# zxhuang1698/ShapeClipper

Measured on AMD Instinct MI355X. Metric: train-step images/sec (Pix3D cfg, bs32/GPU), higher is better.
Workload: dtype f32 (bf16x3-split MFMA, fp32 accumulate)

## Files before the change

### include/shapeclipper_hip.h

```cpp
#ifndef SHAPECLIPPER_HIP_H
#define SHAPECLIPPER_HIP_H
#include <stdint.h>
#ifdef __cplusplus
extern "C" {
#endif

int sc_chamfer3d_forward(const float* xyz1, const float* xyz2, float* dist1, float* dist2,
                         int32_t* idx1, int32_t* idx2, int b, int n, int m, void* stream);

int sc_chamfer3d_forward_split(const float* xyz1, const float* xyz2, float* dist1, float* dist2,
                               int32_t* idx1, int32_t* idx2, int b, int n, int m, int nsplit,
                               void* workspace, void* stream);

long long sc_chamfer3d_grid_workspace_bytes(int b, int n, int m);
int sc_chamfer3d_forward_grid(const float* xyz1, const float* xyz2, float* dist1, float* dist2,
                              int32_t* idx1, int32_t* idx2, int b, int n, int m, void* workspace, void* stream);

int sc_chamfer3d_backward(const float* xyz1, const float* xyz2, float* gradxyz1, float* gradxyz2,
                          const float* graddist1, const float* graddist2, const int32_t* idx1,
                          const int32_t* idx2, int b, int n, int m, void* stream);

long long sc_chamfer3d_backward_ordered_workspace_bytes(int b, int n, int m);
int sc_chamfer3d_backward_ordered_chunk(void);
int sc_chamfer3d_backward_ordered(const float* xyz1, const float* xyz2, float* gradxyz1, float* gradxyz2,
// ... 370 lines not shown
int sc_conv3x3_tile_channels(int hw);
int sc_conv3x3_pack_multi(const long long* table, int n, float* dst, long long total, void* stream);
int sc_conv3x3_pack_multi_units(const long long* table, int n, float* dst, long long total, void* stream);
int sc_conv3x3_pack(const float* w, float* w_pack, int cin, int cout, int hw, int transpose_flip, void* stream);
int sc_conv3x3_forward(const float* x, const float* w_pack, float* out, float* workspace, int batch, int cin, int cout, int hw,
                       void* stream);

long long sc_conv3x3_pack_floats_split(int cin, int cout, int hw);
long long sc_conv3x3_workspace_floats_split(int hw);
int sc_conv3x3_tile_channels_split(int hw);
int sc_conv3x3_forward_split(const float* x, const float* w_pack, float* out, float* workspace, int batch, int cin, int cout, int hw,
                             void* stream);
int sc_conv3x3_forward_add(const float* x, const float* w_pack, const float* addend, float* out, float* workspace, int batch, int cin,
                           int cout, int hw, int split, void* stream);

long long sc_conv3x3s2_bd_pack_floats(int cin, int cout, int hw);
long long sc_conv3x3s2_bd_workspace_floats(int hw);
int sc_conv3x3s2_bd_pack(const float* w, float* w_pack, int cin, int cout, int hw, void* stream);
int sc_conv3x3s2_backward_data(const float* gy, const float* w_pack, float* gx, float* workspace, int batch, int cin, int cout, int hw,
                               void* stream);
int sc_conv3x3s2_wgrad(const float* gy, const float* x, float* dw, float* workspace, int batch, int cin, int cout, int hw, void* stream);
long long sc_conv3x3s2_pack_floats(int cin, int cout, int hw);
long long sc_conv3x3s2_workspace_floats(int hw);
int sc_conv3x3s2_forward(const float* x, const float* w_pack, float* out, float* workspace, int batch, int cin, int cout, int hw,
                         void* stream);

long long sc_conv3x3_wgrad_workspace_floats(int cin, int cout);
int sc_conv3x3_wgrad(const float* gy, const float* x, float* dw, float* workspace, int batch, int cin, int cout, int hw, void* stream);
int sc_conv3x3_wgrad_split(const float* gy, const float* x, float* dw, float* workspace, int batch, int cin, int cout, int hw, void* stream);

long long sc_conv_stem_wgrad_workspace_floats(void);
int sc_conv_stem_forward(const float* x, const float* w, float* out, int batch, void* stream);
int sc_conv_stem_wgrad(const float* gy, const float* x, float* dw, float* workspace, int batch, void* stream);

long long sc_conv1x1s2_wgrad_workspace_floats(int cin, int cout);
int sc_conv1x1s2_forward(const float* x, const float* w, float* out, int batch, int cin, int cout, int hin, void* stream);
int sc_conv1x1s2_backward_data(const float* gy, const float* w, float* gx, int batch, int cin, int cout, int hin, void* stream);
int sc_conv1x1s2_wgrad(const float* gy, const float* x, float* dw, float* workspace, int batch, int cin, int cout, int hin, void* stream);

typedef struct sc_block_args {
    const float *x, *pf1, *pf2, *pb1, *pb2;
    const float *g1, *b1, *g2, *b2;
    float *rm1, *rv1, *rm2, *rv2;
    int64_t *nt1, *nt2;
    float *y1, *a1, *y2, *out, *st1, *st2;
    float *conv_ws, *bn_ws, *wgrad_ws;
    const float* d_out;
    float *dy2, *dres, *da1, *dy1, *dx, *gw1, *gw2, *dgb1, *dgb2;
    int batch, channels, hw, groups, training, split, need_dx;
    float mom1, eps1, mom2, eps2;
} sc_block_args;
int sc_basic_block_forward(const sc_block_args* args, void* stream);
int sc_basic_block_backward(const sc_block_args* args, void* stream);

int sc_linear_bn_supported(int N, int Cin, int Cout, int groups);
int sc_linear_bn_forward(const float* x, const float* w, const float* gamma, const float* beta, const float* res, float* y, float* out,
                         float* save_mean, float* save_rstd, float* run_mean, float* run_var, int64_t* n_tracked, int N, int Cin,
                         int Cout, int groups, int training, int relu, float eps, float momentum, void* stream);
int sc_linear_bn_backward(const float* g_out, const float* gy_next, const float* w_next, const float* g_add, int Cnext, const float* out,
                          const float* y, const float* save_mean, const float* save_rstd, const float* gamma, const float* x, float* gy,
                          float* g_res, float* dw, float* dgamma, float* dbeta, int N, int Cin, int Cout, int groups, int training, int relu,
                          void* stream);
int sc_linear_backward_data(const float* gy, const float* w, const float* g_add, float* dx, int N, int Cin, int Cout, void* stream);

int sc_latent_bias_forward(const float* z, const float* lat, const float* bias, const float* post, float* out, int B, int Z, int L, int NL,
                           void* stream);
// ... 49 lines not shown
```

### shapeclipper_amd/_lib.py

```python
from __future__ import annotations

import ctypes
import os
import re
import threading
from typing import Optional

import torch

_HERE = os.path.dirname(os.path.abspath(__file__))
LIB_PATH = os.environ.get("SHAPECLIPPER_HIP_LIB") or os.path.join(_HERE, "lib", "libshapeclipper_hip.so")

HEADER_PATH = os.path.join(_HERE, os.pardir, "include", "shapeclipper_hip.h")
_CTYPES = {"int": ctypes.c_int, "long long": ctypes.c_longlong, "float": ctypes.c_float, "double": ctypes.c_double}


def read_signatures(text):
    text = re.sub(r"/\*.*?\*/|//[^\n]*", " ", text, flags=re.S)
    text = re.sub(r"^[ \t]*#.*$", " ", text, flags=re.M)
    text = re.sub(r"typedef struct sc_block_args \{.*?\} sc_block_args", " ", text, flags=re.S)
    text = re.sub(r'extern "C" \{|\}', " ", text)
    sigs = {}
    for decl in filter(None, (" ".join(d.split()) for d in text.split(";"))):
        m = re.fullmatch(r"(int|long long) (sc_\w+)\((.*)\)", decl)
        if m is None:
            raise RuntimeError("shapeclipper_amd: include/shapeclipper_hip.h: unrecognised declaration %r" % decl)
        params = [] if m.group(3) == "void" else m.group(3).split(",")
        try:
            args = [ctypes.c_void_p if "*" in p else _CTYPES[" ".join(w for w in p.split()[:-1] if w != "const")] for p in params]
        except KeyError:
            raise RuntimeError("shapeclipper_amd: include/shapeclipper_hip.h: unrecognised parameter type in %r" % decl) from None
        sigs[m.group(2)] = (_CTYPES[m.group(1)], args)
    return sigs


with open(HEADER_PATH) as _f:
    SIGNATURES = read_signatures(_f.read())
SYMBOLS = tuple(n for n, (res, _) in SIGNATURES.items() if res is ctypes.c_int)
SYMBOLS_OTHER = tuple(n for n, (res, _) in SIGNATURES.items() if res is ctypes.c_longlong)

_lib: Optional[ctypes.CDLL] = None

TIMING = None
TIMING_SKIP = ("sc_sdf_stream_pack", "sc_sdf_stream_pack_bytes", "sc_rgb_composite_backward_fused_parts", "sc_rgb_composite_backward_fused_partial_floats", "sc_latent_bias_forward", "sc_latent_bias_backward", "sc_set_reserved_cus", "sc_grid_cus", "sc_chamfer3d_backward_ordered_chunk","sc_conv3x3_release_tables", "sc_linear_bn_supported", "sc_linear_bn_forward", "sc_linear_bn_backward", "sc_linear_backward_data", "sc_bn_splits", "sc_isosurface_blocks_per_image", "sc_marching_cubes_mesh_vertex_blocks_per_image", "sc_bn_act_forward", "sc_bn_act_backward", "sc_bn_relu_pool_forward", "sc_bn_relu_pool_backward",
               "sc_conv3x3_forward", "sc_conv3x3_forward_split", "sc_conv3x3_forward_add", "sc_conv3x3_wgrad", "sc_conv3x3_wgrad_split", "sc_conv3x3_pack", "sc_conv3x3_pack_multi", "sc_conv3x3_pack_multi_units",
               "sc_conv_stem_forward", "sc_conv_stem_wgrad", "sc_conv1x1s2_forward", "sc_conv1x1s2_backward_data", "sc_conv1x1s2_wgrad",
               "sc_conv3x3s2_forward", "sc_conv3x3s2_bd_pack", "sc_conv3x3s2_backward_data", "sc_conv3x3s2_wgrad", "sc_conv3x3_tile_channels", "sc_conv3x3_tile_channels_split",
               "sc_basic_block_forward", "sc_basic_block_backward")

class _Timed:

    def __init__(self, name, fn):
        self.name, self.fn = name, fn

    def __call__(self, *args):
        if TIMING is None:
            return self.fn(*args)
        s, e = torch.cuda.Event(enable_timing=True), torch.cuda.Event(enable_timing=True)
        s.record()
        code = self.fn(*args)
        e.record()
        TIMING.setdefault(self.name, []).append((s, e, args))
        return code


class _LibProxy:

    def __init__(self, cdll):
        self._cdll = cdll
        for name, (restype, argtypes) in SIGNATURES.items():
            fn = getattr(cdll, name)
            fn.restype, fn.argtypes = restype, argtypes
            setattr(self, name, _Timed(name, fn) if restype is ctypes.c_int and name not in TIMING_SKIP else fn)


class HipLibraryMissing(RuntimeError):
    pass


# ... 45 lines not shown
```

### shapeclipper_amd/csrc/conv_stem.hip

```cpp
#include <hip/hip_runtime.h>

#include "grid_cus.hpp"
#include "shapeclipper_hip.h"

namespace sc {

typedef float st_f32x16 __attribute__((ext_vector_type(16)));

constexpr int ST_WI = 224, ST_WO = 112, ST_WP = 230, ST_K = 147, ST_KP = 148, ST_CO = 64;
constexpr int ST_HWI = ST_WI * ST_WI, ST_HWO = ST_WO * ST_WO;
constexpr int SF_PT = 256;
constexpr int SF_ROWS = 13;
constexpr int SF_CH = SF_ROWS * ST_WP;
constexpr int SF_PATCH = 3 * SF_CH;
constexpr int SF_WLD = 96;
constexpr int SF_LDS = ST_KP * SF_WLD + SF_PATCH;
constexpr int SF_NLOAD = (3 * SF_ROWS + 7) / 8;

__global__ __launch_bounds__(512, 1) void conv_stem_fwd_kernel(const float* __restrict__ x, const float* __restrict__ w,
                                                               float* __restrict__ out, int batch) {
    extern __shared__ float4 st_smem[];
    float* Ws = reinterpret_cast<float*>(st_smem);
    float* Xs = Ws + ST_KP * SF_WLD;
    const int tid = threadIdx.x, lane = tid & 63, wave = __builtin_amdgcn_readfirstlane(tid >> 6), half = lane >> 5;
    const int tiles = batch * (ST_HWO / SF_PT), G = gridDim.x, g = blockIdx.x;
    const int t_lo = (int)((long long)g * tiles / G), t_hi = (int)((long long)(g + 1) * tiles / G);

    for (int i = tid; i < ST_KP * SF_WLD; i += 512) {
        const int k = i / SF_WLD, co = i - k * SF_WLD;
        Ws[i] = (k < ST_K && co < ST_CO) ? w[co * ST_K + k] : 0.f;
    }

    float xv[SF_NLOAD][4];
// ... 165 lines not shown
#pragma unroll
            for (int nt = 0; nt < 5; ++nt)
#pragma unroll
                for (int r = 0; r < 16; ++r) acc[nt][r] += R[((cot * 5 + nt) * 16 + r) * 64 + lane];
        }
        __syncthreads();
    }
    if (kq == 0) {
        float* dst = partial + (size_t)g * SW_PART;
#pragma unroll
        for (int nt = 0; nt < 5; ++nt)
#pragma unroll
            for (int r = 0; r < 16; ++r) dst[((cot * 5 + nt) * 16 + r) * 64 + lane] = acc[nt][r];
    }
}

__global__ void conv_stem_wgrad_reduce_kernel(const float* __restrict__ partial, float* __restrict__ dw, int G) {
    const int e = blockIdx.x * blockDim.x + threadIdx.x;
    if (e >= SW_PART) return;
    float s0 = 0.f, s1 = 0.f, s2 = 0.f, s3 = 0.f;
    int gi = 0;
    for (; gi + 3 < G; gi += 4) {
        s0 += partial[(size_t)gi * SW_PART + e];
        s1 += partial[(size_t)(gi + 1) * SW_PART + e];
        s2 += partial[(size_t)(gi + 2) * SW_PART + e];
        s3 += partial[(size_t)(gi + 3) * SW_PART + e];
    }
    for (; gi < G; ++gi) s0 += partial[(size_t)gi * SW_PART + e];
    const int lane = e & 63, r = (e >> 6) & 15, nt = (e >> 10) % 5, cot = e / (5 * 1024);
    const int co = 32 * cot + (r & 3) + 8 * (r >> 2) + 4 * (lane >> 5), k = 32 * nt + (lane & 31);
    if (k < ST_K) dw[co * ST_K + k] = (s0 + s1) + (s2 + s3);
}

static int stem_cus() { return grid_cus(); }

}

extern "C" long long sc_conv_stem_wgrad_workspace_floats(void) { return (long long)sc::stem_cus() * sc::SW_PART; }

extern "C" int sc_conv_stem_forward(const float* x, const float* w, float* out, int batch, void* stream) {
    if (batch <= 0) return (int)hipErrorInvalidValue;
    (void)hipFuncSetAttribute((const void*)sc::conv_stem_fwd_kernel, hipFuncAttributeMaxDynamicSharedMemorySize, sc::SF_LDS * 4);
    hipLaunchKernelGGL(sc::conv_stem_fwd_kernel, dim3(sc::stem_cus()), dim3(512), sc::SF_LDS * 4, (hipStream_t)stream, x, w, out, batch);
    return (int)hipGetLastError();
}

extern "C" int sc_conv_stem_wgrad(const float* gy, const float* x, float* dw, float* workspace, int batch, void* stream) {
    if (batch <= 0) return (int)hipErrorInvalidValue;
    const int G = sc::stem_cus();
    (void)hipFuncSetAttribute((const void*)sc::conv_stem_wgrad_kernel, hipFuncAttributeMaxDynamicSharedMemorySize, sc::SW_LDS * 4);
    hipLaunchKernelGGL(sc::conv_stem_wgrad_kernel, dim3(G), dim3(512), sc::SW_LDS * 4, (hipStream_t)stream, gy, x, workspace, batch);
    hipLaunchKernelGGL(sc::conv_stem_wgrad_reduce_kernel, dim3((sc::SW_PART + 255) / 256), dim3(256), 0, (hipStream_t)stream, workspace, dw, G);
    return (int)hipGetLastError();
}
```

### shapeclipper_amd/functional.py

```python
from __future__ import annotations

import torch

from . import ops


class SdfFunction(torch.autograd.Function):

    @staticmethod
    def forward(ctx, points, w_pack, cbias, n_per_image, symmetric, want_grad, want_feat, fused_backward=True):
        ctx.set_materialize_grads(False)
        points = points.contiguous()
        need = any(ctx.needs_input_grad[:3])
        res = ops.sdf_forward(points, w_pack, cbias, n_per_image, symmetric=symmetric, want_grad=want_grad,
                              want_feat=want_feat, stash=need)
        sdf, grad, feat = res[0], res[1], res[2]
        ctx.meta = (n_per_image, cbias.shape[0], symmetric, want_grad, want_feat)
        ctx.fused_backward = fused_backward
        if need:
            ctx.save_for_backward(points, w_pack, res[3], res[4] if want_grad else None)
        empty = points.new_empty(0)
        outs = (sdf, grad if want_grad else empty, feat if want_feat else empty)
        nd = [o for o, w in zip(outs[1:], (want_grad, want_feat)) if not w]
        if nd:
# ... 228 lines not shown
    return BnReluPoolFunction.apply(x, bn.weight, bn.bias, *_bn_state(bn), groups)


class Conv3x3Function(torch.autograd.Function):

    @staticmethod
    def forward(ctx, x, w, pack_f, pack_b, split):
        x = ops._aligned(x)
        ctx.save_for_backward(x, w, pack_b)
        ctx.split = split
        if pack_f is None:
            pack_f = ops.conv3x3_pack(w, x.shape[2], False, split)
        return ops.conv3x3_apply(x, pack_f, w.shape[0], split)

    @staticmethod
    def backward(ctx, gy):
        x, w, pack_b = ctx.saved_tensors
        gy = ops._aligned(gy)
        gx = None
        if ctx.needs_input_grad[0]:
            gx = ops.conv3x3_apply(gy, pack_b if pack_b is not None else ops.conv3x3_pack(w, x.shape[2], True, ctx.split), w.shape[1], ctx.split)
        gw = None
        if ctx.needs_input_grad[1]:
            if ops.conv3x3_wgrad_supported(x.shape, w.shape):
                gw = ops.conv3x3_backward_weight(gy, x, split=ctx.split)
            else:
                gw = torch.ops.aten.convolution_backward(gy, x, w, None, [1, 1], [1, 1], [1, 1], False, [0, 0], 1, [False, True, False])[1]
        return gx, gw, None, None, None


class ConvStemFunction(torch.autograd.Function):

    @staticmethod
    def forward(ctx, x, w):
        x = ops._aligned(x)
        ctx.save_for_backward(x, w)
        return ops.conv_stem_forward(x, w)

    @staticmethod
    def backward(ctx, gy):
        x, w = ctx.saved_tensors
        gy = ops._aligned(gy)
        gx = None
        if ctx.needs_input_grad[0]:
            gx = torch.ops.aten.convolution_backward(gy, x, w, None, [2, 2], [3, 3], [1, 1], False, [0, 0], 1, [True, False, False])[0]
        gw = ops.conv_stem_backward_weight(gy, x) if ctx.needs_input_grad[1] else None
        return gx, gw


def conv_stem(conv, x):
    if (x.is_cuda and x.dtype == torch.float32 and conv.bias is None and conv.groups == 1 and conv.dilation == (1, 1)
            and ops.conv_stem_supported(x.shape, conv.weight.shape, conv.stride, conv.padding)):
        return ConvStemFunction.apply(x, conv.weight)
    return conv(x)


class Conv1x1S2Function(torch.autograd.Function):

    @staticmethod
    def forward(ctx, x, w):
        x = ops._aligned(x)
        ctx.save_for_backward(x, w)
        return ops.conv1x1s2_forward(x, w)

    @staticmethod
    def backward(ctx, gy):
        x, w = ctx.saved_tensors
        gy = ops._aligned(gy)
        gx = ops.conv1x1s2_backward_data(gy, w) if ctx.needs_input_grad[0] else None
        gw = ops.conv1x1s2_backward_weight(gy, x) if ctx.needs_input_grad[1] else None
        return gx, gw


def conv1x1s2(conv, x):
    if (x.is_cuda and x.dtype == torch.float32 and conv.bias is None and conv.groups == 1 and conv.dilation == (1, 1)
            and ops.conv1x1s2_supported(x.shape, conv.weight.shape, conv.stride, conv.padding)):
        return Conv1x1S2Function.apply(x, conv.weight)
    return conv(x)


class Conv3x3S2Function(torch.autograd.Function):

    @staticmethod
    def forward(ctx, x, w):
        x = ops._aligned(x)
        ctx.save_for_backward(x, w)
# ... 200 lines not shown
```

### shapeclipper_amd/model/resnet.py

```python
from __future__ import annotations

import torch
import torch.nn as nn

from ..functional import basic_block, basic_block_takes, bn_act, bn_relu_maxpool, conv1x1s2, conv3x3, conv3x3s2, conv_stem

FUSED_BN = True
HIP_CONV3X3 = True
HIP_CONV_STEM = True
HIP_CONV3X3_S2 = True
HIP_CONV3X3_S2_GRADS = True
HIP_CONV_1X1 = True
FUSED_BLOCK = True
HIP_CONV3X3_SPLIT = True


class BasicBlock(nn.Module):
    expansion = 1

    def __init__(self, inplanes, planes, stride=1, downsample=None):
        super().__init__()
        self.conv1 = nn.Conv2d(inplanes, planes, 3, stride, 1, bias=False)
        self.bn1 = nn.BatchNorm2d(planes)
        self.relu = nn.ReLU(inplace=True)
        self.conv2 = nn.Conv2d(planes, planes, 3, 1, 1, bias=False)
        self.bn2 = nn.BatchNorm2d(planes)
        self.downsample = downsample

    def forward(self, x, groups=1, packs=None, hip_conv=None):
        if not FUSED_BN:
            assert groups == 1
            identity = x if self.downsample is None else self.downsample(x)
            out = self.relu(self.bn1(self.conv1(x)))
            out = self.bn2(self.conv2(out))
            return self.relu(out + identity)
        use_hip = HIP_CONV3X3 if hip_conv is None else hip_conv
        if use_hip and FUSED_BLOCK and basic_block_takes(self, x, packs):
            return basic_block(self, x, packs, groups)
        identity = x if self.downsample is None else bn_act(
            self.downsample[1], conv1x1s2(self.downsample[0], x) if (use_hip and HIP_CONV_1X1) else self.downsample[0](x), relu=False, groups=groups)
        conv = (lambda m, t: conv3x3s2(m, t) if (m.stride == (2, 2) and HIP_CONV3X3_S2) else conv3x3(m, t, packs)) if use_hip else (lambda m, t: m(t))
        out = bn_act(self.bn1, conv(self.conv1, x), groups=groups)
        return bn_act(self.bn2, conv(self.conv2, out), residual=identity, groups=groups)


class ResNet(nn.Module):
    def __init__(self, layers, num_classes=1000):
# ... 91 lines not shown
```

### shapeclipper_amd/ops.py

```python
from __future__ import annotations

import collections
import ctypes
import weakref

import torch

from . import _lib
from .packing import n_tiles

_SCRATCH = {}


def _scratch(tag, dev, n_floats):
    if dev.type != "cuda":
        raise RuntimeError(_lib.NO_CPU)
    key = (tag, dev.index, torch._C._cuda_getCurrentRawStream(dev.index))
    buf = _SCRATCH.get(key)
    if buf is None or buf.numel() < n_floats:
        buf = _SCRATCH[key] = torch.empty(n_floats, device=dev, dtype=torch.float32)
    return buf


SDF_SCRATCH_FLOATS = 256 * 8 * 5 * 1024
# ... 1021 lines not shown
    code = _lib.load().sc_basic_block_forward(ctypes.byref(a), _lib.raw_stream(x.get_device()))
    if code:
        _lib.check(code, "sc_basic_block_forward")
    return out, (y1, a1, y2, st[0], st[1])


def basic_block_backward(d_out, x, saved, out, pb1, pb2, g1, b1, g2, b2, training, split, groups, need_dx, need_w1, need_w2):
    y1, a1, y2, st1, st2 = saved
    B, C, H, _ = x.shape
    dy2, da1, dy1 = (torch.empty_like(x) for _ in range(3))
    dx, dres = (torch.empty_like(x), torch.empty_like(x)) if need_dx else (None, None)
    gw1 = torch.empty(C, C, 3, 3, device=x.device, dtype=torch.float32) if need_w1 else None
    gw2 = torch.empty(C, C, 3, 3, device=x.device, dtype=torch.float32) if need_w2 else None
    dgb = torch.empty(2, 2, C, device=x.device, dtype=torch.float32)
    a = BlockArgs()
    a.x, a.pb1, a.pb2, a.d_out = x.data_ptr(), pb1.data_ptr(), pb2.data_ptr(), d_out.data_ptr()
    a.g1, a.b1, a.g2, a.b2 = g1.data_ptr(), b1.data_ptr(), g2.data_ptr(), b2.data_ptr()
    a.y1, a.a1, a.y2, a.out, a.st1, a.st2 = y1.data_ptr(), a1.data_ptr(), y2.data_ptr(), out.data_ptr(), st1.data_ptr(), st2.data_ptr()
    a.dy2, a.da1, a.dy1, a.dres, a.dx = dy2.data_ptr(), da1.data_ptr(), dy1.data_ptr(), _p(dres), _p(dx)
    a.gw1, a.gw2, a.dgb1, a.dgb2 = _p(gw1), _p(gw2), dgb[0].data_ptr(), dgb[1].data_ptr()
    a.conv_ws, a.bn_ws = _conv_workspace(x.device, H, split).data_ptr(), _bn_partial(x, groups)
    a.wgrad_ws = _wgrad_workspace(x, C, C).data_ptr() if (need_w1 or need_w2) else None
    a.batch, a.channels, a.hw, a.groups, a.training, a.split, a.need_dx = B, C, H, groups, 1 if training else 0, 1 if split else 0, 1 if need_dx else 0
    code = _lib.load().sc_basic_block_backward(ctypes.byref(a), _lib.raw_stream(x.get_device()))
    if code:
        _lib.check(code, "sc_basic_block_backward")
    return dx, gw1, dgb[0, 0], dgb[0, 1], gw2, dgb[1, 0], dgb[1, 1]


def conv_stem_supported(x_shape, w_shape, stride=2, padding=3) -> bool:
    return (tuple(x_shape[1:]) == (3, 224, 224) and tuple(w_shape) == (64, 3, 7, 7) and stride in (2, (2, 2)) and padding in (3, (3, 3)))


def conv_stem_forward(x, w):
    lib = _lib.load()
    x, w = _aligned(x), _aligned(w)
    out = torch.empty(x.shape[0], 64, 112, 112, device=x.device, dtype=torch.float32)
    _lib.check(lib.sc_conv_stem_forward(_lib.ptr(x), _lib.ptr(w), _lib.ptr(out), x.shape[0], _lib.stream()), "sc_conv_stem_forward")
    return out


def conv_stem_backward_weight(gy, x):
    lib = _lib.load()
    gy, x = _aligned(gy), _aligned(x)
    ws = _scratch("conv stem", x.device, lib.sc_conv_stem_wgrad_workspace_floats())
    dw = torch.empty(64, 3, 7, 7, device=x.device, dtype=torch.float32)
    _lib.check(lib.sc_conv_stem_wgrad(_lib.ptr(gy), _lib.ptr(x), _lib.ptr(dw), _lib.ptr(ws), x.shape[0], _lib.stream()), "sc_conv_stem_wgrad")
    return dw


def conv1x1s2_supported(x_shape, w_shape, stride=2, padding=0) -> bool:
    return (len(x_shape) == 4 and tuple(w_shape[2:]) == (1, 1) and stride in (2, (2, 2)) and padding in (0, (0, 0)) and x_shape[2] == x_shape[3]
            and x_shape[2] % 2 == 0 and w_shape[1] == x_shape[1] and w_shape[0] % 64 == 0 and w_shape[1] % 64 == 0)


def conv1x1s2_forward(x, w):
    lib = _lib.load()
    x, w = _aligned(x), _aligned(w)
    B, cin, H, _ = x.shape
    out = torch.empty(B, w.shape[0], H // 2, H // 2, device=x.device, dtype=torch.float32)
    _lib.check(lib.sc_conv1x1s2_forward(_lib.ptr(x), _lib.ptr(w), _lib.ptr(out), B, cin, w.shape[0], H, _lib.stream()), "sc_conv1x1s2_forward")
    return out


def conv1x1s2_backward_data(gy, w):
    lib = _lib.load()
    gy, w = _aligned(gy), _aligned(w)
    B, cout, Ho, _ = gy.shape
    gx = torch.empty(B, w.shape[1], 2 * Ho, 2 * Ho, device=gy.device, dtype=torch.float32)
    _lib.check(lib.sc_conv1x1s2_backward_data(_lib.ptr(gy), _lib.ptr(w), _lib.ptr(gx), B, w.shape[1], cout, 2 * Ho, _lib.stream()),
               "sc_conv1x1s2_backward_data")
    return gx


def conv1x1s2_backward_weight(gy, x):
    lib = _lib.load()
    gy, x = _aligned(gy), _aligned(x)
    B, cin, H, _ = x.shape
    cout = gy.shape[1]
    n = lib.sc_conv1x1s2_wgrad_workspace_floats(cin, cout)
# ... 886 lines not shown
```

### shapeclipper_amd/utils/options.py

```python
from __future__ import annotations

import collections
import importlib
import os
import random
import string
import sys

import numpy as np
import torch
import yaml

from . import util
from .util import EasyDict as edict
from .util import log

torch.backends.cudnn.benchmark = False

Switch = collections.namedtuple("Switch", ["key", "default", "kind", "text", "drives"])
HIP_TABLE = tuple(Switch(*row) for row in (
    ("device_rng", False, bool, "draw the render's jitter on the GPU (no 4 MB upload per render, another random stream than the reference)", None),
    ("device_choice", True, bool, "pick the regularisation view on the device (reg.n_views = 1)", None),
    ("device_rays", True, bool, "Pix3D: silhouette-weighted ray choice for the whole batch on the GPU (csrc/silhouette_rays.hip)", None),
    ("device_clip_preprocess", True, bool, "Pix3D: CLIP preprocessing on the GPU (csrc/clip_preprocess.hip)", None),
# ... 3 lines not shown
    ("fused_adam", True, bool, "torch's fused Adam on the device", None),
    ("guarded_step", True, bool, "a non-finite loss skips the update on the device; the host raises one step later", None),
    ("batched_encoders", True, bool, "one grouped encoder pass and one grouped estimator pass per step", None),
    ("two_streams", True, bool, "the view estimator runs on a side stream next to the encoders", None),
    ("overlap_allreduce", False, bool, "multi-GPU: the early gradient segment is all-reduced from inside backward", None),
    ("reserve_cus", 0, (0, None), "multi-GPU: persistent convolution grids sized for the device's CUs minus this many", None),
    ("fused_block", True, bool, "one autograd node per stride-1 BasicBlock", ("model.resnet", "FUSED_BLOCK")),
    ("fused_bottleneck", True, bool, "1x1 Bottleneck_Linear blocks as fused launches (csrc/bottleneck.hip)", ("model.view_estimator", "HIP_BOTTLENECK")),
    ("fused_rgb_wgrad", True, bool, "RGB reverse pass forms the weight gradients in the kernel; off: Gy_l / r_l through HBM and sc_wgrad",
     ("ops", "FUSED_RGB_WGRAD")),
    ("rgb_stash", True, bool, "RGB forward parks its hidden activations for the reverse pass; off: the reverse pass recomputes them",
     ("ops", "RGB_STASH")),
    ("value_split", True, bool, "value-only SDF calls (evaluation grid) on the pre-split bf16x3 chain; off: fp32 MFMA", ("ops", "SDF_VALUE_SPLIT")),
    ("rgb_split", True, bool, "RGB network of the forward pass from pre-split bf16x3 fragments; off: fp32 MFMA", ("ops", "RGB_FWD_SPLIT")),
    ("rgb_bwd_split", True, bool, "RGB reverse chain from pre-split transposed fragments; off: fp32 MFMA (see HIP_REQUIRES)",
     ("ops", "RGB_BWD_SPLIT")),
    ("sdf_stream", True, bool, "SDF forward (value, feature, d sdf/dx) from streamed pre-split fragments; off: fp32 MFMA", ("ops", "SDF_FWD_STREAM")),
    ("upload_stream", True, bool, "the CPU-generator draws are copied on a stream of their own, ahead of the render",
     ("model.renderer", "UPLOAD_STREAM")),
    ("rocblas", True, bool, "the small fp32 GEMMs left to torch go through rocBLAS, process-global; off leaves torch's choice alone", None),
    ("conv3x3", True, bool, "3x3 stride-1 trunk convolutions on csrc/conv3x3.hip", ("model.resnet", "HIP_CONV3X3")),
    ("conv3x3_split", True, bool, "... as exact three-piece bf16 operand splits; off: fp32 MFMA throughout", ("model.resnet", "HIP_CONV3X3_SPLIT")),
    ("conv_stem", True, bool, "the 7x7 stride-2 stem convolution on its HIP kernel", ("model.resnet", "HIP_CONV_STEM")),
    ("conv1x1", True, bool, "the 1x1 stride-2 shortcut convolutions on their HIP kernels", ("model.resnet", "HIP_CONV_1X1")),
    ("conv3x3s2", True, bool, "the 3x3 stride-2 convolutions' forward on its HIP kernel", ("model.resnet", "HIP_CONV3X3_S2")),
    ("conv3x3s2_grads", True, bool, "... and their backward-data / weight gradient", ("model.resnet", "HIP_CONV3X3_S2_GRADS")),
    ("train_vis", False, bool, "training-time visualisation on rank 0: turn-table GIFs and periodic dumps", None),
    ("mesh_color", False, bool, "every mesh dump also writes a coloured PLY with vertex normals", None),
    ("largest_component", False, bool, "evaluation keeps the largest connected component of the level grid", None),
    ("surface_render", False, bool, "every per-sample dump also gets a render at the SDF zero crossing (Renderer.render_surface)", None),
    ("surface_refine", 3, (0, 16), "... refinement rounds of the crossing", None),
    ("surface_scale", 1, (1, 4), "... pixels per pixel side", None),
))
HIP = {row.key: row for row in HIP_TABLE}
HIP_REQUIRES = {"rgb_bwd_split": ("rgb_stash", "fused_rgb_wgrad")}
HIP_DEFAULTS = dict(hip={row.key: row.default for row in HIP_TABLE})
_PACKAGE = __name__.rsplit(".", 2)[0]


def hip(opt, key):
    default = HIP[key].default
    return opt.get("hip", {}).get(key, default)


def dual_mesh_reg(opt):
    ev = opt.get("eval", None) or {}
    reg = ev.get("dual_reg", 0.05)
    if isinstance(reg, bool) or not isinstance(reg, (int, float)) or not 0.0 < reg <= 1.0:
        raise ValueError("eval.dual_reg must be a float in (0, 1], got %r" % (reg,))
    return float(reg) if ev.get("dual_mesh", False) else None


def texture_texels(opt, always=False):
    ev = opt.get("eval", None) or {}
    on, texels = ev.get("texture", False), ev.get("texture_texels", 8)
    if not isinstance(on, bool):
        raise ValueError("eval.texture must be a bool, got %r" % (on,))
    if isinstance(texels, bool) or not isinstance(texels, int) or not 4 <= texels <= 32:
        raise ValueError("eval.texture_texels must be an integer in 4..32, got %r" % (texels,))
    return texels if on or always else None


def mesh_render(opt):
    on = (opt.get("eval", None) or {}).get("mesh_render", False)
    if not isinstance(on, bool):
        raise ValueError("eval.mesh_render must be a bool, got %r" % (on,))
    return on
# ... 88 lines not shown


def _ask(question):
    if not sys.stdin or not sys.stdin.isatty():
        return "y"
    ans = None
    while ans not in ("y", "n"):
        ans = input(question)
    return ans


def override_options(opt, opt_over, key_stack=None, safe_check=False):
    for key, value in opt_over.items():
        if isinstance(value, dict):
            opt[key] = override_options(opt.get(key, edict()), value, key_stack=key_stack + [key], safe_check=safe_check)
        else:
            if safe_check and key not in opt:
                if _ask("\"{}\" not found in original opt, add? (y/n) ".format(".".join(key_stack + [key]))) == "n":
                    print("safe exiting...")
                    sys.exit()
            opt[key] = value
    return opt


def set(opt_cmd={}, verbose=True):
    if verbose:
        log.info("setting configurations...")
    opt = load_options(opt_cmd.yaml)
    opt = override_options(opt, opt_cmd, key_stack=[], safe_check=True)
    for k, v in HIP_DEFAULTS.items():
        cur = opt.get(k, edict())
        for kk, vv in v.items():
            cur.setdefault(kk, vv)
        opt[k] = edict(cur)
    process_options(opt)
    if verbose:
        log.options(opt)
    return opt


def process_options(opt):
    if opt.seed is not None:
        random.seed(opt.seed)
        np.random.seed(opt.seed)
        torch.manual_seed(opt.seed)
        if torch.cuda.is_available():
            torch.cuda.manual_seed_all(opt.seed)
    else:
        opt.name += "_{}".format("".join(random.choice(string.ascii_uppercase) for _ in range(4)))
    opt.output_path = "{0}/{1}/{2}".format(opt.output_root, opt.group, opt.name)
    os.makedirs(opt.output_path, exist_ok=True)
    assert isinstance(opt.gpu, int)
    opt.device = "cpu" if opt.cpu or not torch.cuda.is_available() else "cuda:{}".format(opt.gpu)
    opt.H, opt.W = opt.image_size
    if "data" in opt and "dataset" in opt.data and opt.data.dataset not in opt.data and "pix3d" in opt.data:
        opt.data[opt.data.dataset] = opt.data.pix3d
    for row in HIP_TABLE:
        if row.kind is not bool and None not in row.kind:
            (lo, hi), v = row.kind, hip(opt, row.key)
            if isinstance(v, bool) or not isinstance(v, int) or not lo <= v <= hi:
                raise ValueError("hip.%s must be an integer in %d..%d, got %r" % (row.key, lo, hi, v))
    dual_mesh_reg(opt)
    texture_texels(opt)
    mesh_render(opt)
    icp_settings(opt)
    normal_settings(opt)
    mesh_dist_settings(opt)
    emd_settings(opt)
    iou_settings(opt)
    torch.backends.cudnn.deterministic = bool(hip(opt, "deterministic_conv"))
    for row in HIP_TABLE:
        if row.drives is not None:
            module, attr = row.drives
            on = all(bool(hip(opt, k)) for k in (row.key,) + HIP_REQUIRES.get(row.key, ()))
            setattr(importlib.import_module("%s.%s" % (_PACKAGE, module)), attr, on)
    if bool(hip(opt, "rocblas")) and torch.cuda.is_available():
        try:
            torch.backends.cuda.preferred_blas_library("cublas")
        except Exception:
            pass


def save_options_file(opt):
    fname = "{}/options.yaml".format(opt.output_path)
    if os.path.isfile(fname):
        with open(fname) as f:
            old = yaml.safe_load(f)
        if util.to_dict(opt) != old:
            print("existing options file found (different from current one)...")
            if _ask("override? (y/n) ") == "n":
                print("safe exiting...")
                sys.exit()
        else:
            print("existing options file found (identical)")
    else:
        print("(creating new options file...)")
    with open(fname, "w") as f:
        yaml.safe_dump(util.to_dict(opt), f, default_flow_style=False, indent=4)
```

Measured before the change: 1040.

## Add bf16x3-split MFMA kernels for stem conv forward and weight gradient

Adds new 7x7 stride-2 stem convolution kernels for the forward pass and the weight gradient. Each fp32 operand is split into three bf16 pieces, and the kernels run six bf16 32x32x16 MFMAs per product instead of using fp32 MFMA. The kernels lay out the split pieces in LDS and double-buffer tile loads; the wgrad kernel also reduces partial sums in LDS across waves. A new default-on switch routes the stem through these kernels when conv3x3_split is on, trading the extra split arithmetic and a small precision change for higher MFMA throughput.

```diff
diff --git a/include/shapeclipper_hip.h b/include/shapeclipper_hip.h
--- a/include/shapeclipper_hip.h
+++ b/include/shapeclipper_hip.h
@@ -426,6 +426,8 @@
 long long sc_conv_stem_wgrad_workspace_floats(void);
 int sc_conv_stem_forward(const float* x, const float* w, float* out, int batch, void* stream);
 int sc_conv_stem_wgrad(const float* gy, const float* x, float* dw, float* workspace, int batch, void* stream);
+int sc_conv_stem_forward_split(const float* x, const float* w, float* out, int batch, void* stream);
+int sc_conv_stem_wgrad_split(const float* gy, const float* x, float* dw, float* workspace, int batch, void* stream);
 
 long long sc_conv1x1s2_wgrad_workspace_floats(int cin, int cout);
 int sc_conv1x1s2_forward(const float* x, const float* w, float* out, int batch, int cin, int cout, int hin, void* stream);
diff --git a/shapeclipper_amd/_lib.py b/shapeclipper_amd/_lib.py
--- a/shapeclipper_amd/_lib.py
+++ b/shapeclipper_amd/_lib.py
@@ -44,7 +44,7 @@
 TIMING = None
 TIMING_SKIP = ("sc_sdf_stream_pack", "sc_sdf_stream_pack_bytes", "sc_rgb_composite_backward_fused_parts", "sc_rgb_composite_backward_fused_partial_floats", "sc_latent_bias_forward", "sc_latent_bias_backward", "sc_set_reserved_cus", "sc_grid_cus", "sc_chamfer3d_backward_ordered_chunk","sc_conv3x3_release_tables", "sc_linear_bn_supported", "sc_linear_bn_forward", "sc_linear_bn_backward", "sc_linear_backward_data", "sc_bn_splits", "sc_isosurface_blocks_per_image", "sc_marching_cubes_mesh_vertex_blocks_per_image", "sc_bn_act_forward", "sc_bn_act_backward", "sc_bn_relu_pool_forward", "sc_bn_relu_pool_backward",
                "sc_conv3x3_forward", "sc_conv3x3_forward_split", "sc_conv3x3_forward_add", "sc_conv3x3_wgrad", "sc_conv3x3_wgrad_split", "sc_conv3x3_pack", "sc_conv3x3_pack_multi", "sc_conv3x3_pack_multi_units",
-               "sc_conv_stem_forward", "sc_conv_stem_wgrad", "sc_conv1x1s2_forward", "sc_conv1x1s2_backward_data", "sc_conv1x1s2_wgrad",
+               "sc_conv_stem_forward", "sc_conv_stem_wgrad", "sc_conv_stem_forward_split", "sc_conv_stem_wgrad_split", "sc_conv1x1s2_forward", "sc_conv1x1s2_backward_data", "sc_conv1x1s2_wgrad",
                "sc_conv3x3s2_forward", "sc_conv3x3s2_bd_pack", "sc_conv3x3s2_backward_data", "sc_conv3x3s2_wgrad", "sc_conv3x3_tile_channels", "sc_conv3x3_tile_channels_split",
                "sc_basic_block_forward", "sc_basic_block_backward")
 
diff --git a/shapeclipper_amd/csrc/conv_stem.hip b/shapeclipper_amd/csrc/conv_stem.hip
--- a/shapeclipper_amd/csrc/conv_stem.hip
+++ b/shapeclipper_amd/csrc/conv_stem.hip
@@ -1,4 +1,6 @@
 #include <hip/hip_runtime.h>
+
+#include <type_traits>
 
 #include "grid_cus.hpp"
 #include "shapeclipper_hip.h"
@@ -230,6 +232,305 @@
     if (k < ST_K) dw[co * ST_K + k] = (s0 + s1) + (s2 + s3);
 }
 
+typedef __bf16 st_bf16x8 __attribute__((ext_vector_type(8)));
+typedef unsigned st_u32x4 __attribute__((ext_vector_type(4)));
+
+typedef float st_f32x2 __attribute__((ext_vector_type(2)));
+typedef __bf16 st_bf16x2 __attribute__((ext_vector_type(2)));
+
+__device__ __forceinline__ void st_split2(float lo, float hi, unsigned (&p)[3]) {
+    st_f32x2 r{lo, hi};
+#pragma unroll
+    for (int q = 0; q < 3; ++q) {
+        p[q] = __builtin_bit_cast(unsigned, __builtin_convertvector(r, st_bf16x2));
+        if (q < 2) r -= st_f32x2{__uint_as_float(p[q] << 16), __uint_as_float(p[q] & 0xffff0000u)};
+    }
+}
+template <int NA, int NB>
+__device__ __forceinline__ void st_six(const st_u32x4 (&a)[NA][3], const st_u32x4 (&b)[NB][3], st_f32x16* acc) {
+    constexpr int PA[6] = {0, 2, 1, 0, 1, 0}, PB[6] = {2, 0, 1, 1, 0, 0};
+#pragma unroll
+    for (int t = 0; t < 6; ++t)
+#pragma unroll
+        for (int i = 0; i < NA; ++i)
+#pragma unroll
+            for (int j = 0; j < NB; ++j)
+                acc[i * NB + j] = __builtin_amdgcn_mfma_f32_32x32x16_bf16(__builtin_bit_cast(st_bf16x8, a[i][PA[t]]), __builtin_bit_cast(st_bf16x8, b[j][PB[t]]),
+                                                                          acc[i * NB + j], 0, 0, 0);
+#pragma unroll
+    for (int i = 0; i < NA; ++i)
+#pragma unroll
+        for (int j = 0; j < NB; ++j)
+            asm("" : "+v"(acc[i * NB + j]) : "v"(a[i][0]), "v"(a[i][1]), "v"(a[i][2]), "v"(b[j][0]), "v"(b[j][1]), "v"(b[j][2]));
+}
+
+constexpr int SS_R = 22;
+constexpr int SS_WP = SS_R * ST_CO;
+constexpr int SS_LINE = ST_WP / 2;
+constexpr int SS_XP = 3 * SF_ROWS * SS_LINE;
+constexpr int SS_LDS = 3 * SS_WP * 16 + 3 * SS_XP * 4;
+
+__global__ __launch_bounds__(512, 1) void conv_stem_fwd_split_kernel(const float* __restrict__ x, const float* __restrict__ w,
+                                                                     float* __restrict__ out, int batch) {
+    extern __shared__ float4 st_smem[];
+    st_u32x4* Wq = reinterpret_cast<st_u32x4*>(st_smem);
+    unsigned* Xq = reinterpret_cast<unsigned*>(Wq + 3 * SS_WP);
+    const int tid = threadIdx.x, lane = tid & 63, wave = __builtin_amdgcn_readfirstlane(tid >> 6), half = lane >> 5;
+    const int tiles = batch * (ST_HWO / SF_PT), G = gridDim.x, g = blockIdx.x;
+    const int t_lo = (int)((long long)g * tiles / G), t_hi = (int)((long long)(g + 1) * tiles / G);
+
+    for (int i = tid; i < SS_WP; i += 512) {
+        const int R = i / ST_CO, co = i - R * ST_CO;
+        unsigned pk[3][4] = {};
+        if (R < 21) {
+#pragma unroll
+            for (int j = 0; j < 8; j += 2) {
+                unsigned p[3];
+                st_split2(w[co * ST_K + R * 7 + j], j + 1 < 7 ? w[co * ST_K + R * 7 + j + 1] : 0.f, p);
+#pragma unroll
+                for (int q = 0; q < 3; ++q) pk[q][j >> 1] = p[q];
+            }
+        }
+#pragma unroll
+        for (int q = 0; q < 3; ++q) Wq[q * SS_WP + i] = st_u32x4{pk[q][0], pk[q][1], pk[q][2], pk[q][3]};
+    }
+
+    float xv[SF_NLOAD][2][2];
+    auto load = [&](int tile) {
+        const int b = tile / (ST_HWO / SF_PT), p0 = (tile - b * (ST_HWO / SF_PT)) * SF_PT;
+        const int r0 = 2 * (p0 / ST_WO) - 3;
+        const float* xb = x + (size_t)b * 3 * ST_HWI;
+#pragma unroll
+        for (int l = 0; l < SF_NLOAD; ++l) {
+            const int line = wave + 8 * l, ci = line / SF_ROWS, row = r0 + line - ci * SF_ROWS;
+            const bool row_ok = line < 3 * SF_ROWS && row >= 0 && row < ST_WI;
+#pragma unroll
+            for (int c = 0; c < 2; ++c)
+#pragma unroll
+                for (int e = 0; e < 2; ++e) {
+                    const int col = 2 * (lane + 64 * c) + e - 3;
+                    xv[l][c][e] = (row_ok && col >= 0 && col < ST_WI) ? xb[ci * ST_HWI + row * ST_WI + col] : 0.f;
+                }
+        }
+    };
+    auto store = [&]() {
+#pragma unroll
+        for (int l = 0; l < SF_NLOAD; ++l) {
+            const int line = wave + 8 * l;
+            if (line < 3 * SF_ROWS) {
+#pragma unroll
+                for (int c = 0; c < 2; ++c)
+                    if (lane + 64 * c < SS_LINE) {
+                        unsigned p[3];
+                        st_split2(xv[l][c][0], xv[l][c][1], p);
+#pragma unroll
+                        for (int q = 0; q < 3; ++q) Xq[q * SS_XP + line * SS_LINE + lane + 64 * c] = p[q];
+                    }
+            }
+        }
+    };
+
+    if (t_lo < t_hi) load(t_lo);
+    for (int tile = t_lo; tile < t_hi; ++tile) {
+        __syncthreads();
+        store();
+        __syncthreads();
+        if (tile + 1 < t_hi) load(tile + 1);
+        const int b = tile / (ST_HWO / SF_PT), p0 = (tile - b * (ST_HWO / SF_PT)) * SF_PT;
+        const int p = p0 + wave * 32 + (lane & 31), y = p / ST_WO, xo = p - y * ST_WO;
+        const unsigned* Bb = Xq + (y - p0 / ST_WO) * 2 * SS_LINE + xo;
+        const st_u32x4* Ab = Wq + half * ST_CO + (lane & 31);
+        st_f32x16 acc[2];
+#pragma unroll
+        for (int r = 0; r < 16; ++r) acc[0][r] = acc[1][r] = 0.f;
+        st_u32x4 a[2][2][3], bf[2][1][3];
+        auto frags = [&](int s, st_u32x4 (&af)[2][3], st_u32x4 (&bq)[1][3]) {
+            const int R0 = 2 * s, R1 = 2 * s + 1 < 21 ? 2 * s + 1 : 2 * s;
+            const int o0 = ((R0 / 7) * SF_ROWS + R0 % 7) * SS_LINE, o1 = ((R1 / 7) * SF_ROWS + R1 % 7) * SS_LINE;
+            const unsigned* bp = Bb + o0 + half * (o1 - o0);
+            const unsigned keep = (2 * s + 1 < 21 || !half) ? 0xffffffffu : 0u;
+#pragma unroll
+            for (int q = 0; q < 3; ++q) {
+                bq[0][q] = st_u32x4{bp[q * SS_XP] & keep, bp[q * SS_XP + 1] & keep, bp[q * SS_XP + 2] & keep, bp[q * SS_XP + 3] & keep & 0xffffu};
+                af[0][q] = Ab[q * SS_WP + 2 * s * ST_CO];
+                af[1][q] = Ab[q * SS_WP + 2 * s * ST_CO + 32];
+            }
+        };
+        frags(0, a[0], bf[0]);
+#pragma unroll
+        for (int s = 0; s < SS_R / 2; ++s) {
+            if (s + 1 < SS_R / 2) frags(s + 1, a[(s + 1) & 1], bf[(s + 1) & 1]);
+            st_six<2, 1>(a[s & 1], bf[s & 1], acc);
+        }
+        float* ob = out + (size_t)b * ST_CO * ST_HWO + p;
+#pragma unroll
+        for (int i = 0; i < 2; ++i)
+#pragma unroll
+            for (int r = 0; r < 16; ++r) ob[(size_t)(32 * i + (r & 3) + 8 * (r >> 2) + 4 * half) * ST_HWO] = acc[i][r];
+    }
+}
+
+constexpr int SV_PL = 58;
+constexpr int SV_XP = 2 * 3 * SW_ROWS * SV_PL;
+constexpr int SV_GST = 29 * 4;
+constexpr int SV_GP = ST_CO * SV_GST;
+constexpr int SV_GOFF = 3 * SV_XP;
+static_assert(SV_GOFF % 4 == 0, "the gy image is read with ds_read_b128");
+constexpr int SV_LDS = (SV_GOFF + 3 * SV_GP) * 4;
+static_assert(3 * SV_GP >= SW_PART && SV_LDS <= 160 * 1024, "the gy image also holds one partial block in the final sum");
+
+__global__ __launch_bounds__(512, 1) void conv_stem_wgrad_split_kernel(const float* __restrict__ gy, const float* __restrict__ x,
+                                                                       float* __restrict__ partial, int batch) {
+    extern __shared__ float4 st_smem[];
+    unsigned* Xq = reinterpret_cast<unsigned*>(st_smem);
+    unsigned* Gq = Xq + SV_GOFF;
+    const int tid = threadIdx.x, lane = tid & 63, wave = __builtin_amdgcn_readfirstlane(tid >> 6), half = lane >> 5;
+    const int cot = wave & 1, kq = wave >> 1;
+    const int steps = batch * (ST_WO / 2), G = gridDim.x, g = blockIdx.x;
+    const int s_lo = (int)((long long)g * steps / G), s_hi = (int)((long long)(g + 1) * steps / G);
+
+    for (int i = tid; i < SV_LDS / 4; i += 512) Xq[i] = 0u;
+
+    float xv[4][4], gv[8][4];
+    auto load = [&](int step) {
+        const int b = step / (ST_WO / 2), y0 = 2 * (step - b * (ST_WO / 2));
+        const float* xb = x + (size_t)b * 3 * ST_HWI;
+#pragma unroll
+        for (int l = 0; l < 4; ++l) {
+            const int line = wave + 8 * l, ci = line / SW_ROWS, row = 2 * y0 - 3 + line - ci * SW_ROWS;
+            const bool row_ok = line < 3 * SW_ROWS && row >= 0 && row < ST_WI;
+#pragma unroll
+            for (int c = 0; c < 4; ++c) {
+                const int col = 4 * lane + c - 3;
+                xv[l][c] = (row_ok && col >= 0 && col < ST_WI && 4 * lane + c < ST_WP) ? xb[ci * ST_HWI + row * ST_WI + col] : 0.f;
+            }
+        }
+        const float* gb = gy + ((size_t)b * ST_CO + 8 * wave) * ST_HWO + y0 * ST_WO;
+#pragma unroll
+        for (int ch = 0; ch < 8; ++ch)
+#pragma unroll
+            for (int c = 0; c < 2; ++c) {
+                const bool ok = lane + 64 * c < ST_WO;
+                const float2 v = ok ? *reinterpret_cast<const float2*>(gb + ch * ST_HWO + 2 * (lane + 64 * c)) : make_float2(0.f, 0.f);
+                gv[ch][2 * c] = v.x, gv[ch][2 * c + 1] = v.y;
+            }
+    };
+    auto store = [&]() {
+#pragma unroll
+        for (int l = 0; l < 4; ++l) {
+            const int line = wave + 8 * l;
+            if (line < 3 * SW_ROWS && lane < SV_PL) {
+                unsigned ev[3], od[3];
+                st_split2(xv[l][0], xv[l][2], ev);
+                st_split2(xv[l][1], xv[l][3], od);
+#pragma unroll
+                for (int q = 0; q < 3; ++q) {
+                    Xq[q * SV_XP + line * SV_PL + lane] = ev[q];
+                    Xq[q * SV_XP + (3 * SW_ROWS + line) * SV_PL + lane] = od[q];
+                }
+            }
+        }
+#pragma unroll
+        for (int ch = 0; ch < 8; ++ch)
+#pragma unroll
+            for (int c = 0; c < 2; ++c)
+                if (lane + 64 * c < ST_WO) {
+                    unsigned p[3];
+                    st_split2(gv[ch][2 * c], gv[ch][2 * c + 1], p);
+#pragma unroll
+                    for (int q = 0; q < 3; ++q) Gq[q * SV_GP + (8 * wave + ch) * SV_GST + lane + 64 * c] = p[q];
+                }
+    };
+
+    int tapb[5];
+    unsigned tsh[5];
+#pragma unroll
+    for (int nt = 0; nt < 5; ++nt) {
+        const int k = 32 * nt + (lane & 31), kx = k % 7, q = kx >> 1;
+        tapb[nt] = k < ST_K ? ((kx & 1) * 3 * SW_ROWS + (k / 49) * SW_ROWS + (k % 49) / 7) * SV_PL + (q >> 1) + 4 * half : 4 * half;
+        tsh[nt] = k < ST_K ? 16u * (q & 1) : 0u;
+    }
+    const st_u32x4* Ab = reinterpret_cast<const st_u32x4*>(Gq + (32 * cot + (lane & 31)) * SV_GST) + half;
+
+    st_f32x16 acc[5];
+#pragma unroll
+    for (int nt = 0; nt < 5; ++nt)
+#pragma unroll
+        for (int r = 0; r < 16; ++r) acc[nt][r] = 0.f;
+
+    const int g_lo = kq < 2 ? 4 * kq : 3 * kq + 2, g_n = kq < 2 ? 4 : 3;
+    if (s_lo < s_hi) load(s_lo);
+    __syncthreads();
+    for (int step = s_lo; step < s_hi; ++step) {
+        store();
+        __syncthreads();
+        if (step + 1 < s_hi) load(step + 1);
+#pragma unroll
+        for (int gi = 0; gi < 4; ++gi) {
+            if (gi < g_n) {
+                const int grp = g_lo + gi;
+                const int r = grp / 7, x0 = (grp - 7 * r) * 16;
+                st_u32x4 a[1][3];
+#pragma unroll
+                for (int q = 0; q < 3; ++q) a[0][q] = Ab[q * (SV_GP / 4) + (r * ST_WO + x0) / 8];
+                const int po = r * 2 * SV_PL + x0 / 2;
+                auto tiles = [&](auto nb, int nt0) {
+                    constexpr int NB = decltype(nb)::value;
+                    unsigned d[NB][3][5];
+#pragma unroll
+                    for (int j = 0; j < NB; ++j) {
+                        const unsigned* bp = Xq + tapb[nt0 + j] + po;
+#pragma unroll
+                        for (int q = 0; q < 3; ++q)
+#pragma unroll
+                            for (int e = 0; e < 5; ++e) d[j][q][e] = bp[q * SV_XP + e];
+                    }
+                    __builtin_amdgcn_sched_barrier(0);
+                    st_u32x4 bf[NB][3];
+#pragma unroll
+                    for (int j = 0; j < NB; ++j) {
+                        const unsigned sh = tsh[nt0 + j];
+#pragma unroll
+                        for (int q = 0; q < 3; ++q)
+                            bf[j][q] = st_u32x4{__builtin_amdgcn_alignbit(d[j][q][1], d[j][q][0], sh), __builtin_amdgcn_alignbit(d[j][q][2], d[j][q][1], sh),
+                                                __builtin_amdgcn_alignbit(d[j][q][3], d[j][q][2], sh), __builtin_amdgcn_alignbit(d[j][q][4], d[j][q][3], sh)};
+                    }
+                    st_six<1, NB>(a, bf, acc + nt0);
+                };
+                tiles(std::integral_constant<int, 3>{}, 0);
+                tiles(std::integral_constant<int, 2>{}, 3);
+            }
+        }
+        __syncthreads();
+    }
+
+    float* R = reinterpret_cast<float*>(Gq);
+#pragma unroll 1
+    for (int q = 1; q < 4; ++q) {
+        if (kq == q) {
+#pragma unroll
+            for (int nt = 0; nt < 5; ++nt)
+#pragma unroll
+                for (int r = 0; r < 16; ++r) R[((cot * 5 + nt) * 16 + r) * 64 + lane] = acc[nt][r];
+        }
+        __syncthreads();
+        if (kq == 0) {
+#pragma unroll
+            for (int nt = 0; nt < 5; ++nt)
+#pragma unroll
+                for (int r = 0; r < 16; ++r) acc[nt][r] += R[((cot * 5 + nt) * 16 + r) * 64 + lane];
+        }
+        __syncthreads();
+    }
+    if (kq == 0) {
+        float* dst = partial + (size_t)g * SW_PART;
+#pragma unroll
+        for (int nt = 0; nt < 5; ++nt)
+#pragma unroll
+            for (int r = 0; r < 16; ++r) dst[((cot * 5 + nt) * 16 + r) * 64 + lane] = acc[nt][r];
+    }
+}
+
 static int stem_cus() { return grid_cus(); }
 
 }
@@ -240,6 +541,13 @@
     if (batch <= 0) return (int)hipErrorInvalidValue;
     (void)hipFuncSetAttribute((const void*)sc::conv_stem_fwd_kernel, hipFuncAttributeMaxDynamicSharedMemorySize, sc::SF_LDS * 4);
     hipLaunchKernelGGL(sc::conv_stem_fwd_kernel, dim3(sc::stem_cus()), dim3(512), sc::SF_LDS * 4, (hipStream_t)stream, x, w, out, batch);
+    return (int)hipGetLastError();
+}
+
+extern "C" int sc_conv_stem_forward_split(const float* x, const float* w, float* out, int batch, void* stream) {
+    if (batch <= 0) return (int)hipErrorInvalidValue;
+    (void)hipFuncSetAttribute((const void*)sc::conv_stem_fwd_split_kernel, hipFuncAttributeMaxDynamicSharedMemorySize, sc::SS_LDS);
+    hipLaunchKernelGGL(sc::conv_stem_fwd_split_kernel, dim3(sc::stem_cus()), dim3(512), sc::SS_LDS, (hipStream_t)stream, x, w, out, batch);
     return (int)hipGetLastError();
 }
 
@@ -251,3 +559,12 @@
     hipLaunchKernelGGL(sc::conv_stem_wgrad_reduce_kernel, dim3((sc::SW_PART + 255) / 256), dim3(256), 0, (hipStream_t)stream, workspace, dw, G);
     return (int)hipGetLastError();
 }
+
+extern "C" int sc_conv_stem_wgrad_split(const float* gy, const float* x, float* dw, float* workspace, int batch, void* stream) {
+    if (batch <= 0) return (int)hipErrorInvalidValue;
+    const int G = sc::stem_cus();
+    (void)hipFuncSetAttribute((const void*)sc::conv_stem_wgrad_split_kernel, hipFuncAttributeMaxDynamicSharedMemorySize, sc::SV_LDS);
+    hipLaunchKernelGGL(sc::conv_stem_wgrad_split_kernel, dim3(G), dim3(512), sc::SV_LDS, (hipStream_t)stream, gy, x, workspace, batch);
+    hipLaunchKernelGGL(sc::conv_stem_wgrad_reduce_kernel, dim3((sc::SW_PART + 255) / 256), dim3(256), 0, (hipStream_t)stream, workspace, dw, G);
+    return (int)hipGetLastError();
+}
diff --git a/shapeclipper_amd/functional.py b/shapeclipper_amd/functional.py
--- a/shapeclipper_amd/functional.py
+++ b/shapeclipper_amd/functional.py
@@ -284,10 +284,11 @@
 class ConvStemFunction(torch.autograd.Function):
 
     @staticmethod
-    def forward(ctx, x, w):
+    def forward(ctx, x, w, split=False):
         x = ops._aligned(x)
         ctx.save_for_backward(x, w)
-        return ops.conv_stem_forward(x, w)
+        ctx.split = split
+        return ops.conv_stem_forward(x, w, split=split)
 
     @staticmethod
     def backward(ctx, gy):
@@ -296,14 +297,15 @@
         gx = None
         if ctx.needs_input_grad[0]:
             gx = torch.ops.aten.convolution_backward(gy, x, w, None, [2, 2], [3, 3], [1, 1], False, [0, 0], 1, [True, False, False])[0]
-        gw = ops.conv_stem_backward_weight(gy, x) if ctx.needs_input_grad[1] else None
-        return gx, gw
+        gw = ops.conv_stem_backward_weight(gy, x, split=ctx.split) if ctx.needs_input_grad[1] else None
+        return gx, gw, None
 
 
 def conv_stem(conv, x):
     if (x.is_cuda and x.dtype == torch.float32 and conv.bias is None and conv.groups == 1 and conv.dilation == (1, 1)
             and ops.conv_stem_supported(x.shape, conv.weight.shape, conv.stride, conv.padding)):
-        return ConvStemFunction.apply(x, conv.weight)
+        from .model import resnet
+        return ConvStemFunction.apply(x, conv.weight, bool(resnet.HIP_CONV3X3_SPLIT and resnet.HIP_STEM_SPLIT))
     return conv(x)
 
 
diff --git a/shapeclipper_amd/model/resnet.py b/shapeclipper_amd/model/resnet.py
--- a/shapeclipper_amd/model/resnet.py
+++ b/shapeclipper_amd/model/resnet.py
@@ -13,6 +13,7 @@
 HIP_CONV_1X1 = True
 FUSED_BLOCK = True
 HIP_CONV3X3_SPLIT = True
+HIP_STEM_SPLIT = True
 
 
 class BasicBlock(nn.Module):
diff --git a/shapeclipper_amd/ops.py b/shapeclipper_amd/ops.py
--- a/shapeclipper_amd/ops.py
+++ b/shapeclipper_amd/ops.py
@@ -1077,20 +1077,22 @@
     return (tuple(x_shape[1:]) == (3, 224, 224) and tuple(w_shape) == (64, 3, 7, 7) and stride in (2, (2, 2)) and padding in (3, (3, 3)))
 
 
-def conv_stem_forward(x, w):
+def conv_stem_forward(x, w, split=False):
     lib = _lib.load()
     x, w = _aligned(x), _aligned(w)
     out = torch.empty(x.shape[0], 64, 112, 112, device=x.device, dtype=torch.float32)
-    _lib.check(lib.sc_conv_stem_forward(_lib.ptr(x), _lib.ptr(w), _lib.ptr(out), x.shape[0], _lib.stream()), "sc_conv_stem_forward")
+    name = "sc_conv_stem_forward_split" if split else "sc_conv_stem_forward"
+    _lib.check(getattr(lib, name)(_lib.ptr(x), _lib.ptr(w), _lib.ptr(out), x.shape[0], _lib.stream()), name)
     return out
 
 
-def conv_stem_backward_weight(gy, x):
+def conv_stem_backward_weight(gy, x, split=False):
     lib = _lib.load()
     gy, x = _aligned(gy), _aligned(x)
     ws = _scratch("conv stem", x.device, lib.sc_conv_stem_wgrad_workspace_floats())
     dw = torch.empty(64, 3, 7, 7, device=x.device, dtype=torch.float32)
-    _lib.check(lib.sc_conv_stem_wgrad(_lib.ptr(gy), _lib.ptr(x), _lib.ptr(dw), _lib.ptr(ws), x.shape[0], _lib.stream()), "sc_conv_stem_wgrad")
+    name = "sc_conv_stem_wgrad_split" if split else "sc_conv_stem_wgrad"
+    _lib.check(getattr(lib, name)(_lib.ptr(gy), _lib.ptr(x), _lib.ptr(dw), _lib.ptr(ws), x.shape[0], _lib.stream()), name)
     return dw
 
 
diff --git a/shapeclipper_amd/utils/options.py b/shapeclipper_amd/utils/options.py
--- a/shapeclipper_amd/utils/options.py
+++ b/shapeclipper_amd/utils/options.py
@@ -59,7 +59,11 @@
     ("surface_refine", 3, (0, 16), "... refinement rounds of the crossing", None),
     ("surface_scale", 1, (1, 4), "... pixels per pixel side", None),
 ))
-HIP = {row.key: row for row in HIP_TABLE}
+HIP_REFINEMENTS = (
+    Switch("stem_split", True, bool, "the stem's forward / weight gradient as exact three-piece bf16 operand splits while conv3x3_split is on; "
+           "off: fp32 MFMA", ("model.resnet", "HIP_STEM_SPLIT")),
+)
+HIP = {row.key: row for row in HIP_TABLE + HIP_REFINEMENTS}
 HIP_REQUIRES = {"rgb_bwd_split": ("rgb_stash", "fused_rgb_wgrad")}
 HIP_DEFAULTS = dict(hip={row.key: row.default for row in HIP_TABLE})
 _PACKAGE = __name__.rsplit(".", 2)[0]
@@ -214,6 +218,8 @@
         cur = opt.get(k, edict())
         for kk, vv in v.items():
             cur.setdefault(kk, vv)
+        for row in HIP_REFINEMENTS:
+            cur.setdefault(row.key, row.default)
         opt[k] = edict(cur)
     process_options(opt)
     if verbose:
@@ -251,7 +257,7 @@
     emd_settings(opt)
     iou_settings(opt)
     torch.backends.cudnn.deterministic = bool(hip(opt, "deterministic_conv"))
-    for row in HIP_TABLE:
+    for row in HIP_TABLE + HIP_REFINEMENTS:
         if row.drives is not None:
             module, attr = row.drives
             on = all(bool(hip(opt, k)) for k in (row.key,) + HIP_REQUIRES.get(row.key, ()))
```

After: 1023. 0.983x the previous value.
